# Ghostish/Open3DSOT

Measured on NVIDIA H100. Metric: template-search pairs/sec, BAT-Car fwd+bwd, higher is better.
Workload: dtype f32

## Files before the change

open3dsot_b200/csrc/pwmlp_tc.cu:

```cuda
#include "common.cuh"
#include "lift.cuh"
#include "tc_ptx.cuh"
#include "../../include/o3d_b200.h"

namespace {

struct TcAct {
    const float* x; int ld; const float* scale; const float* shift; int relu;
    struct Coef { float4 s, t; bool on; };
    template <int R> struct Batch { float4 v[R]; };
    __device__ __forceinline__ Coef prep(int k, int K) const {
        Coef c;
        c.on = k < K;
        c.s = make_float4(1.f, 1.f, 1.f, 1.f);
        c.t = make_float4(0.f, 0.f, 0.f, 0.f);
        if (c.on && scale) { c.s = ld4g(scale + k); c.t = ld4g(shift + k); }
        return c;
    }
    template <int R>
    __device__ __forceinline__ void fetch(Batch<R>& b, int p0, int stride, int P, int k, int K) const {
        const int kk = k < K ? k : 0;
#pragma unroll
        for (int i = 0; i < R; ++i) {
            const int p = p0 + i * stride;
            b.v[i] = ld4g(x + (size_t)(p < P ? p : P - 1) * ld + kk);
        }
    }
    template <int R>
    __device__ __forceinline__ float4 finish(const Batch<R>& b, const Coef& c, int i, int p, int P) const {
        float4 v = b.v[i];
        if (!(c.on && p < P)) return make_float4(0.f, 0.f, 0.f, 0.f);
        if (scale) { v.x = fmaf(v.x, c.s.x, c.t.x); v.y = fmaf(v.y, c.s.y, c.t.y); v.z = fmaf(v.z, c.s.z, c.t.z); v.w = fmaf(v.w, c.s.w, c.t.w); }
        if (relu) { v.x = fmaxf(v.x, 0.f); v.y = fmaxf(v.y, 0.f); v.z = fmaxf(v.z, 0.f); v.w = fmaxf(v.w, 0.f); }
        return v;
    }
    __device__ __forceinline__ void prefetch_rows(int p0, int rows, int P) const {
        if (p0 < P) o3d_prefetch_l2(x + (size_t)p0 * ld, (size_t)min(rows, P - p0) * ld * sizeof(float));
    }
};

struct TcLift {
    LiftView lv; const float* scale; const float* shift; int relu;
    int la;
    struct Coef { float4 s, t, u0, u1, u2, u3; bool on; };
    template <int R> struct Batch { float4 v[R]; float4 sv[R]; int nrow[R]; int tag; };
    __device__ __forceinline__ Coef prep(int k, int K) const {
        Coef c;
        c.on = k < K;
        c.s = make_float4(1.f, 1.f, 1.f, 1.f);
        c.t = c.u0 = c.u1 = c.u2 = c.u3 = make_float4(0.f, 0.f, 0.f, 0.f);
        if (c.on && scale) { c.s = ld4g(scale + k); c.t = ld4g(shift + k); }
        if (c.on && lv.u) { c.u0 = ld4g(lv.u + k); c.u1 = ld4g(lv.u + lv.ldz + k); c.u2 = ld4g(lv.u + 2 * lv.ldz + k); c.u3 = ld4g(lv.u + 3 * lv.ldz + k); }
        return c;
    }
    template <int R>
    __device__ __forceinline__ void fetch(Batch<R>& b, int p0, int stride, int P, int k, int K) const {
        const int kk = k < K ? k : 0;
        if (lv.z) {
            int row[R];
            if (b.tag == p0 + 1) {
#pragma unroll
                for (int i = 0; i < R; ++i) row[i] = b.nrow[i];
            } else if (R == 4 && stride == 1 && (p0 & 3) == 0 && p0 + 3 < P) {
                const int4 r4 = __ldg(reinterpret_cast<const int4*>(lv.gidx + p0));
                row[0] = r4.x; row[R > 1 ? 1 : 0] = r4.y; row[R > 2 ? 2 : 0] = r4.z; row[R > 3 ? 3 : 0] = r4.w;
            } else {
#pragma unroll
                for (int i = 0; i < R; ++i) {
                    const int p = p0 + i * stride;
                    row[i] = __ldg(lv.gidx + (p < P ? p : P - 1));
                }
            }
#pragma unroll
            for (int i = 0; i < R; ++i) b.v[i] = ld4g(lv.z + (size_t)row[i] * lv.ldz + kk);
            if (la == 0) {
#pragma unroll
                for (int i = 0; i < R; ++i) b.nrow[i] = row[i];
                b.tag = p0 + 1;
            } else {
                const int pn = p0 + la;
#pragma unroll
                for (int i = 0; i < R; ++i) {
                    const int p = pn + i * stride;
                    b.nrow[i] = __ldg(lv.gidx + (p < P ? p : P - 1));
                }
                b.tag = pn + 1;
            }
        }
        if (lv.s) {
#pragma unroll
            for (int i = 0; i < R; ++i) {
                const int p = p0 + i * stride;
                b.sv[i] = ld4g(lv.s + (size_t)(p < P ? p : P - 1) * 4);
            }
        }
    }
    template <int R>
    __device__ __forceinline__ float4 finish(const Batch<R>& b, const Coef& c, int i, int p, int P) const {
        const float4 zero = make_float4(0.f, 0.f, 0.f, 0.f);
        if (!(c.on && p < P)) return zero;
        float4 v = lift_val4(lv.z ? b.v[i] : zero, lv.s ? b.sv[i] : zero, c.u0, c.u1, c.u2, c.u3);
        if (scale) { v.x = fmaf(v.x, c.s.x, c.t.x); v.y = fmaf(v.y, c.s.y, c.t.y); v.z = fmaf(v.z, c.s.z, c.t.z); v.w = fmaf(v.w, c.s.w, c.t.w); }
        if (relu) { v.x = fmaxf(v.x, 0.f); v.y = fmaxf(v.y, 0.f); v.z = fmaxf(v.z, 0.f); v.w = fmaxf(v.w, 0.f); }
        return v;
    }
    __device__ __forceinline__ void prefetch_rows(int p0, int rows, int P) const {
        if (p0 >= P) return;
        const size_t n = (size_t)min(rows, P - p0);
        if (lv.z) o3d_prefetch_l2(lv.gidx + p0, n * sizeof(int32_t));
        if (lv.s) o3d_prefetch_l2(lv.s + (size_t)p0 * 4, n * 16);
    }
};

struct TcDy {
    const float* g; int ldg; const float* y; int ldy; const float* a; const float* b; const float* cc;
    const float* dpool; const int32_t* sel; int S; int ldp;
    int sh;
    int dbg;
    struct Coef { float4 a, b, c; bool on; };
    template <int R> struct Batch { float4 g[R]; float4 y[R]; bool shared; };
    __device__ __forceinline__ Coef prep(int k, int K) const {
        Coef c;
        c.on = k < K;
        c.a = make_float4(1.f, 1.f, 1.f, 1.f);
        c.b = c.c = make_float4(0.f, 0.f, 0.f, 0.f);
        if (c.on && a) { c.a = ld4g(a + k); c.b = ld4g(b + k); c.c = ld4g(cc + k); }
        return c;
    }
    template <int R>
    __device__ __forceinline__ void fetch(Batch<R>& bt, int p0, int stride, int P, int k, int K) const {
        const int kk = k < K ? k : 0;
        bt.shared = false;
        if (dpool) {
            const int pf = p0 < P ? p0 : P - 1;
            const int pe = p0 + (R - 1) * stride;
            const int pl = pe < P ? pe : P - 1;
            if (R >= 2 && (pf >> sh) == (pl >> sh)) {
                bt.shared = true;
                const size_t go = (size_t)(pf >> sh) * ldp + kk;
                if (!(dbg & 256)) {
                    bt.g[0] = ld4g(dpool + go);
                    const int4 sl = __ldg(reinterpret_cast<const int4*>(sel + go));
                    bt.g[R >= 2 ? 1 : 0] = make_float4(__int_as_float(sl.x), __int_as_float(sl.y), __int_as_float(sl.z), __int_as_float(sl.w));
                } else {
                    bt.g[0] = bt.g[R >= 2 ? 1 : 0] = make_float4(0.f, 0.f, 0.f, 0.f);
                }
            } else {
#pragma unroll
                for (int i = 0; i < R; ++i) {
                    const int p = p0 + i * stride, pp = p < P ? p : P - 1;
                    const int s = pp & (S - 1);
                    const size_t go = (size_t)(pp >> sh) * ldp + kk;
                    const int4 sl = __ldg(reinterpret_cast<const int4*>(sel + go));
                    const float4 d = ld4g(dpool + go);
                    bt.g[i] = make_float4(sl.x == s ? d.x : 0.f, sl.y == s ? d.y : 0.f, sl.z == s ? d.z : 0.f, sl.w == s ? d.w : 0.f);
                }
            }
        } else {
#pragma unroll
            for (int i = 0; i < R; ++i) {
                const int p = p0 + i * stride;
                bt.g[i] = ld4g(g + (size_t)(p < P ? p : P - 1) * ldg + kk);
            }
        }
#pragma unroll
        for (int i = 0; i < R; ++i) {
            const int p = p0 + i * stride;
            bt.y[i] = (a && !(dbg & 512)) ? ld4g(y + (size_t)(p < P ? p : P - 1) * ldy + kk) : make_float4(0.f, 0.f, 0.f, 0.f);
        }
    }
    template <int R>
    __device__ __forceinline__ float4 finish(const Batch<R>& bt, const Coef& c, int i, int p, int P) const {
        if (!(c.on && p < P)) return make_float4(0.f, 0.f, 0.f, 0.f);
        float4 v = bt.g[i];
        if (bt.shared) {
            const int s = p & (S - 1);
            const float4 d = bt.g[0], sl = bt.g[R >= 2 ? 1 : 0];
            v = make_float4(__float_as_int(sl.x) == s ? d.x : 0.f, __float_as_int(sl.y) == s ? d.y : 0.f,
                            __float_as_int(sl.z) == s ? d.z : 0.f, __float_as_int(sl.w) == s ? d.w : 0.f);
        }
        if (a) {
            const float4 yy = bt.y[i];
            v.x = fmaf(c.a.x, v.x, fmaf(c.c.x, yy.x, c.b.x)); v.y = fmaf(c.a.y, v.y, fmaf(c.c.y, yy.y, c.b.y));
            v.z = fmaf(c.a.z, v.z, fmaf(c.c.z, yy.z, c.b.z)); v.w = fmaf(c.a.w, v.w, fmaf(c.c.w, yy.w, c.b.w));
        }
        return v;
    }
    __device__ __forceinline__ void prefetch_rows(int p0, int rows, int P) const {
        if (p0 >= P) return;
        const size_t n = (size_t)min(rows, P - p0);
        if (!dpool) o3d_prefetch_l2(g + (size_t)p0 * ldg, n * ldg * sizeof(float));
        if (a) o3d_prefetch_l2(y + (size_t)p0 * ldy, n * ldy * sizeof(float));
        if (dpool) {
            const int g0 = p0 >> sh, g1 = (p0 + (int)n - 1) >> sh;
            const size_t bytes = (size_t)(g1 - g0 + 1) * ldp * sizeof(float);
            o3d_prefetch_l2(dpool + (size_t)g0 * ldp, bytes);
            o3d_prefetch_l2(sel + (size_t)g0 * ldp, bytes);
        }
    }
};

template <int LD>
struct TcFwdEpi {
    float* y; int ldy; const float* bias; double* sum; double* sumsq;
    int S, log2S; float* ymax; float* ymin; int32_t* arg; int ldp;
    float bv, mx, mn; int ax, an; double d1, d2;
    __device__ __forceinline__ void begin(int ch, int Nw) {
        d1 = d2 = 0.0;
        bv = (bias && ch < Nw) ? bias[ch] : 0.f;
        mx = -INFINITY; mn = INFINITY; ax = an = 0;
    }
    __device__ __forceinline__ void prefetch(int, int, int, int) {}
    __device__ __forceinline__ const int32_t* lift_gidx() const { return nullptr; }
    __device__ __forceinline__ const float* lift_s() const { return nullptr; }
    __device__ __forceinline__ void set_tile(const int32_t*, const float4*) {}
    __device__ __forceinline__ void group(const uint32_t (&r)[16], int ch, int Nw, int pbase, int P) {
        if (ch >= Nw) return;
        float s1 = 0.f, s2 = 0.f;
        const int smask = S - 1;
        float* yp = y ? y + (size_t)pbase * ldy + ch : nullptr;
        if (pbase + 16 <= P && (S == 0 || S >= 16)) {
            float v[16];
#pragma unroll
            for (int j = 0; j < 16; ++j) v[j] = __uint_as_float(r[j]) + bv;
            if (yp) {
                const size_t st = LD ? (size_t)LD : (size_t)ldy;
#pragma unroll
                for (int j = 0; j < 16; ++j) yp[j * st] = v[j];
            }
#pragma unroll
            for (int j = 0; j < 16; ++j) {
                s1 += v[j];
                s2 = fmaf(v[j], v[j], s2);
            }
            if (S > 0) {
                float gm = v[0], gn = v[0];
                int ga = 0, gb = 0;
#pragma unroll
                for (int j = 1; j < 16; ++j) {
                    if (v[j] > gm) { gm = v[j]; ga = j; }
                    if (v[j] < gn) { gn = v[j]; gb = j; }
                }
                const int s0 = pbase & smask;
                if (s0 == 0) { mx = gm; ax = ga; mn = gn; an = gb; }
                else {
                    if (gm > mx) { mx = gm; ax = s0 + ga; }
                    if (gn < mn) { mn = gn; an = s0 + gb; }
                }
                if (s0 + 16 == S) {
                    const size_t o = (size_t)(pbase >> log2S) * ldp + ch;
                    ymax[o] = mx; ymin[o] = mn; arg[o] = ax | (an << 16);
                }
            }
        } else {
#pragma unroll
            for (int j = 0; j < 16; ++j) {
                if (pbase + j >= P) break;
                const float v = __uint_as_float(r[j]) + bv;
                if (yp) yp[(size_t)j * ldy] = v;
                s1 += v;
                s2 = fmaf(v, v, s2);
                if (S > 0) {
                    const int s = (pbase + j) & smask;
                    if (s == 0) { mx = -INFINITY; mn = INFINITY; ax = an = 0; }
                    if (v > mx) { mx = v; ax = s; }
                    if (v < mn) { mn = v; an = s; }
                    if (s == smask) {
                        const size_t o = (size_t)((pbase + j) >> log2S) * ldp + ch;
                        ymax[o] = mx; ymin[o] = mn; arg[o] = ax | (an << 16);
                    }
                }
            }
        }
        d1 += (double)s1;
        d2 += (double)s2;
    }
    __device__ __forceinline__ void end(int ch, int Nw) {
        if (sum && ch < Nw) {
            atomicAdd(sum + ch, d1);
            atomicAdd(sumsq + ch, d2);
        }
    }
};

template <int LD, bool LIFT = false>
struct TcDgradEpi {
    float* out; int ldo; const float* yprev; int ldyp; const float* scale; const float* shift; int relu;
    double* s1g; double* s2y;
    LiftView lv;
    float sc, sh; double d1, d2;
    float yv[16];
    float u0, u1, u2, u3; const int32_t* gs; const float4* ss;
    __device__ __forceinline__ bool lifted() const { return LIFT; }
    __device__ __forceinline__ void begin(int ch, int Nw) {
        d1 = d2 = 0.0;
        sc = (scale && ch < Nw) ? scale[ch] : 1.f;
        sh = (shift && ch < Nw) ? shift[ch] : 0.f;
        if constexpr (LIFT) {
            const bool on = lv.u && ch < Nw;
            u0 = on ? lv.u[ch] : 0.f; u1 = on ? lv.u[lv.ldz + ch] : 0.f; u2 = on ? lv.u[2 * lv.ldz + ch] : 0.f; u3 = on ? lv.u[3 * lv.ldz + ch] : 0.f;
            gs = nullptr;
        }
    }
    __device__ __forceinline__ const int32_t* lift_gidx() const { return LIFT ? lv.gidx : nullptr; }
    __device__ __forceinline__ const float* lift_s() const { return LIFT ? lv.s : nullptr; }
    __device__ __forceinline__ void set_tile(const int32_t* g, const float4* s4) { if constexpr (LIFT) { gs = g; ss = s4; } }
    __device__ __forceinline__ void prefetch_lift(int ch, int pbase, int col, int P) {
#pragma unroll
        for (int j = 0; j < 16; ++j) {
            const float z = lv.z ? __ldg(lv.z + (size_t)gs[col + j] * lv.ldz + ch) : 0.f;
            const float4 sv = lv.s ? ss[col + j] : make_float4(0.f, 0.f, 0.f, 0.f);
            yv[j] = lift_val(z, sv, u0, u1, u2, u3);
        }
    }
    __device__ __forceinline__ void prefetch(int ch, int Nw, int pbase, int P) {
        if (ch >= Nw) return;
        if constexpr (LIFT) { prefetch_lift(ch, pbase, pbase & (TC_N - 1), P); return; }
        if (!yprev) return;
        if (pbase + 16 <= P) {
            const float* yp = yprev + (size_t)pbase * ldyp + ch;
            const size_t st = LD ? (size_t)LD : (size_t)ldyp;
#pragma unroll
            for (int j = 0; j < 16; ++j) yv[j] = __ldg(yp + j * st);
        } else {
#pragma unroll
            for (int j = 0; j < 16; ++j) {
                const int pj = min(pbase + j, P - 1);
                yv[j] = __ldg(yprev + (size_t)pj * ldyp + ch);
            }
        }
    }
    __device__ __forceinline__ void group(const uint32_t (&r)[16], int ch, int Nw, int pbase, int P) {
        if (ch >= Nw) return;
        float s1 = 0.f, s2 = 0.f;
        float* op = out + (size_t)pbase * ldo + ch;
        if (pbase + 16 <= P) {
            float v[16];
#pragma unroll
            for (int j = 0; j < 16; ++j) v[j] = __uint_as_float(r[j]);
            if (yprev || lifted()) {
                if (relu) {
#pragma unroll
                    for (int j = 0; j < 16; ++j) v[j] = fmaf(yv[j], sc, sh) > 0.f ? v[j] : 0.f;
                }
#pragma unroll
                for (int j = 0; j < 16; ++j) s2 = fmaf(v[j], yv[j], s2);
            }
            const size_t st = LD ? (size_t)LD : (size_t)ldo;
#pragma unroll
            for (int j = 0; j < 16; ++j) {
                s1 += v[j];
                op[j * st] = v[j];
            }
        } else {
#pragma unroll
            for (int j = 0; j < 16; ++j) {
                if (pbase + j >= P) break;
                float v = __uint_as_float(r[j]);
                if (yprev || lifted()) {
                    if (relu && !(fmaf(yv[j], sc, sh) > 0.f)) v = 0.f;
                    s2 = fmaf(v, yv[j], s2);
                }
                s1 += v;
                op[(size_t)j * ldo] = v;
            }
        }
        d1 += (double)s1;
        d2 += (double)s2;
    }
    __device__ __forceinline__ void end(int ch, int Nw) {
        if (s1g && ch < Nw) {
            atomicAdd(s1g + ch, d1);
            atomicAdd(s2y + ch, d2);
        }
    }
};

constexpr int TC_STAGES = 2;
constexpr int TC_STAGE_BYTES = 4 * TILE_BYTES;
constexpr int TC_EPI_LD = 68;
constexpr int TC_EPI_BYTES = TC_M * TC_EPI_LD * 4;
constexpr int TC_THREADS = 512;
constexpr int TC_SMEM = TC_STAGES * TC_STAGE_BYTES + 2 * TC_EPI_BYTES + 1024 + 256 + 1024 + 4096;

template <int R>
__device__ __forceinline__ void stage_acc(const float (&acc)[R], float* stg, int ld) {
    const int w = (threadIdx.x >> 5) & 3, lane = threadIdx.x & 31;
#pragma unroll
    for (int i = 0; i < R; ++i) {
        const int row = 16 * w + (lane >> 2) + 8 * ((i >> 1) & 1), col = 8 * (i >> 2) + 2 * (lane & 3) + (i & 1);
        stg[col * ld + row] = acc[i];
    }
}

template <class BLoad, class Epi>
__global__ void __launch_bounds__(TC_THREADS, 1)
    pw_tc_kernel(BLoad bl, const uint8_t* __restrict__ wtiles, int P, int K, int Nw, int nkb, Epi epi, int dbg, int rev) {
    extern __shared__ uint8_t smem_raw[];
    uint8_t* smem = reinterpret_cast<uint8_t*>((reinterpret_cast<uintptr_t>(smem_raw) + 1023) & ~(uintptr_t)1023);
    uint8_t* tail = smem + TC_STAGES * TC_STAGE_BYTES + 2 * TC_EPI_BYTES;
    uint64_t* full = reinterpret_cast<uint64_t*>(tail);
    uint64_t* empty = full + TC_STAGES;

    const int warp = threadIdx.x >> 5, lane = threadIdx.x & 31;
    const int mt0 = blockIdx.y;
    const int n_ptiles = (P + TC_N - 1) / TC_N;
    auto tile_of = [&](int t) { return rev ? n_ptiles - 1 - t : t; };

    if (threadIdx.x == 0) {
        for (int s = 0; s < TC_STAGES; ++s) {
            o3d_mbar_init(full + s, 256 + 1);
            o3d_mbar_init(empty + s, 8);
        }
        o3d_fence_mbar_init();
    }
    __syncthreads();

    if (warp < 8) {
        const int h = warp >> 2;
        const int tw = threadIdx.x & 127;
        const int ch = mt0 * TC_M + tw;
        float* stg = reinterpret_cast<float*>(smem + TC_STAGES * TC_STAGE_BYTES + h * TC_EPI_BYTES);
        int32_t* gsm = reinterpret_cast<int32_t*>(tail + 256);
        float4* ssm = reinterpret_cast<float4*>(tail + 256 + 1024);
        epi.begin(ch, Nw);
        const int Nw_e = (dbg & 4) ? 0 : Nw;
        int stage = 0, phase = 0, buf = 0;
        for (int t = blockIdx.x; t < n_ptiles; t += gridDim.x) {
            const int pt0 = tile_of(t) * TC_N;
            {
                const int32_t* gi = epi.lift_gidx();
                const float* si = epi.lift_s();
                if (gi || si) {
                    const int pp = min(pt0 + tw, P - 1);
                    if (gi && h == 0) gsm[buf * TC_N + tw] = __ldg(gi + pp);
                    if (si && h == 1) ssm[buf * TC_N + tw] = ld4g(si + (size_t)pp * 4);
                    asm volatile("bar.sync 1, 256;" ::: "memory");
                    epi.set_tile(gsm + buf * TC_N, ssm + buf * TC_N);
                }
            }
            const int pb = pt0 + h * 64;
            epi.prefetch(ch, Nw_e, pb, P);
            float acc[64];
#pragma unroll
            for (int i = 0; i < 64; ++i) acc[i] = 0.f;
            for (int kb = 0; kb < nkb; ++kb) {
                o3d_mbar_wait(full + stage, phase);
                const uint32_t sb = o3d_smem_u32(smem + stage * TC_STAGE_BYTES);
                const uint32_t xb = sb + 2 * TILE_BYTES + h * (TILE_BYTES / 2);
                wgmma_fence_acc(acc);
                wgmma_fence();
                wgmma_3xtf32_kblock<128>(acc, make_desc(xb), make_desc(xb + TILE_BYTES), make_desc(sb), make_desc(sb + TILE_BYTES),
                                         kb == 0);
                wgmma_commit();
                wgmma_wait<0>();
                wgmma_fence_acc(acc);
                if (lane == 0) o3d_mbar_arrive(empty + stage);
                if (++stage == TC_STAGES) { stage = 0; phase ^= 1; }
            }
            asm volatile("bar.sync %0, 128;" ::"r"(2 + h) : "memory");
            stage_acc(acc, stg, TC_EPI_LD);
            asm volatile("bar.sync %0, 128;" ::"r"(2 + h) : "memory");
            const float* row = stg + tw * TC_EPI_LD;
#pragma unroll 1
            for (int cg = 0; cg < 4; ++cg) {
                uint32_t r[16];
#pragma unroll
                for (int j = 0; j < 4; ++j) {
                    const float4 v = *reinterpret_cast<const float4*>(row + cg * 16 + 4 * j);
                    r[4 * j] = __float_as_uint(v.x); r[4 * j + 1] = __float_as_uint(v.y);
                    r[4 * j + 2] = __float_as_uint(v.z); r[4 * j + 3] = __float_as_uint(v.w);
                }
                epi.group(r, ch, Nw_e, pb + cg * 16, P);
                if (cg + 1 < 4) epi.prefetch(ch, Nw_e, pb + (cg + 1) * 16, P);
            }
            buf ^= 1;
        }
        epi.end(ch, Nw);
    } else {
        const int pt = (warp - 8) * 32 + lane;
        const int chunk = pt & 7;
        const int row0 = (pt >> 3) * 4;
        int stage = 0, phase = 0;
        if (dbg & 2) P = 0;
        struct Cur { int t, kb, p0; };
        auto advance = [&](Cur& c) {
            if (++c.kb == nkb) {
                c.kb = 0;
                c.t += gridDim.x;
                if (c.t < n_ptiles) c.p0 = tile_of(c.t) * TC_N;
            }
        };
        using Batch4 = typename BLoad::template Batch<4>;
        auto issue = [&](Batch4& r, typename BLoad::Coef& cf, const Cur& c) {
            if (c.t >= n_ptiles) return;
            const int k = c.kb * TC_K + chunk * 4;
            cf = bl.prep(k, K);
            if (P > 0) bl.fetch(r, c.p0 + row0, 1, P, k, K);
        };
        Cur c0{(int)blockIdx.x, 0, 0};
        if (c0.t < n_ptiles) c0.p0 = tile_of(c0.t) * TC_N;
        Batch4 r0{};
        typename BLoad::Coef f0 = bl.prep(chunk * 4, K);
        issue(r0, f0, c0);
        if (pt == 0 && c0.t < n_ptiles) bl.prefetch_rows(c0.p0, TC_N, P);
        while (c0.t < n_ptiles) {
            o3d_mbar_wait(empty + stage, phase ^ 1);
            if (pt == 0) {
                o3d_mbar_expect_tx(full + stage, 2 * TILE_BYTES);
                o3d_bulk_g2s(smem + stage * TC_STAGE_BYTES, wtiles + ((size_t)mt0 * nkb + c0.kb) * (2 * TILE_BYTES), 2 * TILE_BYTES,
                             full + stage);
                const int tn = c0.t + (int)gridDim.x;
                if (c0.kb == 0 && tn < n_ptiles) bl.prefetch_rows(tile_of(tn) * TC_N, TC_N, P);
            }
            uint8_t* xhi = smem + stage * TC_STAGE_BYTES + 2 * TILE_BYTES;
            uint8_t* xlo = xhi + TILE_BYTES;
#pragma unroll
            for (int i = 0; i < 4; ++i) {
                const float4 v = P > 0 ? bl.finish(r0, f0, i, c0.p0 + row0 + i, P) : make_float4(0.f, 0.f, 0.f, 0.f);
                const uint32_t off = sw128(row0 + i, chunk);
                *reinterpret_cast<float4*>(xhi + off) = hi_part(v);
                *reinterpret_cast<float4*>(xlo + off) = lo_part(v);
            }
            o3d_fence_proxy_async();
            o3d_mbar_arrive(full + stage);
            if (++stage == TC_STAGES) { stage = 0; phase ^= 1; }
            advance(c0);
            issue(r0, f0, c0);
        }
    }
}

constexpr int WG_STAGES = 3;
constexpr int WG_AHEAD = 4;
constexpr int WG_THREADS = 512;
constexpr int WG_SMEM = WG_STAGES * 4 * TILE_BYTES + 1024 + 256;

template <class L>
__device__ __forceinline__ void store_transposed(const L& ld, const typename L::template Batch<4>& raw, const typename L::Coef& cf,
                                                 uint8_t* hi, int c_local, int p_first, int prow0, int pend) {
#pragma unroll
    for (int i = 0; i < 4; ++i) {
        const int pl = prow0 + 8 * i;
        const float4 v = ld.finish(raw, cf, i, p_first + pl, pend);
        const float e[4] = {v.x, v.y, v.z, v.w};
#pragma unroll
        for (int j = 0; j < 4; ++j) {
            const uint32_t off = sw128(c_local + j, pl >> 2) + (uint32_t)((pl & 3) * 4);
            const float h = hi1(e[j]);
            *reinterpret_cast<float*>(hi + off) = h;
            *reinterpret_cast<float*>(hi + TILE_BYTES + off) = e[j] - h;
        }
    }
}

template <class XB>
__global__ void __launch_bounds__(WG_THREADS, 1)
    pw_wgrad_tc_kernel(TcDy da, XB xb, int P, int M, int N, int chunk, float* __restrict__ dW, int lddw, float* __restrict__ part,
                       int dbg) {
    extern __shared__ uint8_t smem_raw[];
    uint8_t* smem = reinterpret_cast<uint8_t*>((reinterpret_cast<uintptr_t>(smem_raw) + 1023) & ~(uintptr_t)1023);
    uint64_t* full = reinterpret_cast<uint64_t*>(smem + WG_STAGES * 4 * TILE_BYTES);
    uint64_t* empty = full + WG_STAGES;

    const int warp = threadIdx.x >> 5, lane = threadIdx.x & 31;
    const int m0 = blockIdx.z * TC_M, n0 = blockIdx.y * TC_N;
    const int pbeg = blockIdx.x * chunk, pend = min(P, pbeg + chunk);
    const int nkb = pend > pbeg ? (pend - pbeg + TC_K - 1) / TC_K : 0;
    auto kpos = [&](int i) { return pbeg + i * TC_K; };

    if (threadIdx.x == 0) {
        for (int s = 0; s < WG_STAGES; ++s) {
            o3d_mbar_init(full + s, 256);
            o3d_mbar_init(empty + s, 8);
        }
        o3d_fence_mbar_init();
    }
    __syncthreads();

    if (warp < 8) {
        const int h = warp >> 2, w = warp & 3;
        float acc[64];
#pragma unroll
        for (int i = 0; i < 64; ++i) acc[i] = 0.f;
        int stage = 0, phase = 0;
        for (int kb = 0; kb < nkb; ++kb) {
            o3d_mbar_wait(full + stage, phase);
            const uint32_t sb = o3d_smem_u32(smem + stage * 4 * TILE_BYTES);
            const uint32_t ab = sb + h * (TILE_BYTES / 2);
            wgmma_fence_acc(acc);
            wgmma_fence();
            if (!(dbg & 32))
                wgmma_3xtf32_kblock<128>(acc, make_desc(ab), make_desc(ab + TILE_BYTES), make_desc(sb + 2 * TILE_BYTES),
                                         make_desc(sb + 3 * TILE_BYTES), kb == 0);
            wgmma_commit();
            wgmma_wait<0>();
            wgmma_fence_acc(acc);
            if (lane == 0) o3d_mbar_arrive(empty + stage);
            if (++stage == WG_STAGES) { stage = 0; phase ^= 1; }
        }
        const int Mt = TC_M * (int)gridDim.z, Nt = TC_N * (int)gridDim.y;
        float* __restrict__ out = part ? part + (size_t)blockIdx.x * Mt * Nt : nullptr;
#pragma unroll
        for (int i = 0; i < 64; i += 4) {
#pragma unroll
            for (int rr = 0; rr < 2; ++rr) {
                const int m = m0 + h * 64 + 16 * w + (lane >> 2) + 8 * rr, n = n0 + 8 * (i >> 2) + 2 * (lane & 3);
                const float v0 = acc[i + 2 * rr], v1 = acc[i + 2 * rr + 1];
                if (out) {
                    *reinterpret_cast<float2*>(out + (size_t)m * Nt + n) = make_float2(v0, v1);
                } else if (nkb > 0 && m < M) {
                    if (n < N) atomicAdd(dW + (size_t)m * lddw + n, v0);
                    if (n + 1 < N) atomicAdd(dW + (size_t)m * lddw + n + 1, v1);
                }
            }
        }
    } else {
        const int pw = warp - 8;
        const int c4 = pw * 4 + (lane & 3), prow0 = lane >> 2;
        const bool pt0 = pw == 0 && lane == 0;
        TcDy::Batch<4> ra = {};
        typename XB::template Batch<4> rb = {};
        auto fetch = [&](int kb) {
            if (dbg & 2) return;
            da.fetch(ra, kpos(kb) + prow0, 8, pend, m0 + c4 * 4, M);
            xb.fetch(rb, kpos(kb) + prow0, 8, pend, n0 + c4 * 4, N);
        };
        auto prefetch = [&](int kb) {
            if (pt0 && kb < nkb) {
                da.prefetch_rows(kpos(kb), TC_K, pend);
                xb.prefetch_rows(kpos(kb), TC_K, pend);
            }
        };
        int stage = 0, phase = 0;
        for (int kb = 0; kb < WG_AHEAD; ++kb) prefetch(kb);
        if (nkb > 0) fetch(0);
        for (int kb = 0; kb < nkb; ++kb) {
            prefetch(kb + WG_AHEAD);
            o3d_mbar_wait(empty + stage, phase ^ 1);
            uint8_t* sbase = smem + stage * 4 * TILE_BYTES;
            store_transposed(da, ra, da.prep(m0 + c4 * 4, M), sbase, c4 * 4, kpos(kb), prow0, pend);
            store_transposed(xb, rb, xb.prep(n0 + c4 * 4, N), sbase + 2 * TILE_BYTES, c4 * 4, kpos(kb), prow0, pend);
            o3d_fence_proxy_async();
            o3d_mbar_arrive(full + stage);
            if (kb + 1 < nkb) fetch(kb + 1);
            if (++stage == WG_STAGES) { stage = 0; phase ^= 1; }
        }
    }
}

__global__ void __launch_bounds__(256)
    wgrad_reduce_kernel(const float* __restrict__ part, int splits, int Mt, int Nt, int M, int N, float* __restrict__ dW,
                        int lddw) {
    const int sub = threadIdx.x & 7;
    const int n4 = (blockIdx.x * 32 + (threadIdx.x >> 3)) * 4, m = blockIdx.y;
    float4 acc = make_float4(0.f, 0.f, 0.f, 0.f);
    if (n4 < N && m < M) {
        const float* p = part + (size_t)m * Nt + n4;
        for (int s = sub; s < splits; s += 8) {
            const float4 v = __ldg(reinterpret_cast<const float4*>(p + (size_t)s * Mt * Nt));
            acc.x += v.x; acc.y += v.y; acc.z += v.z; acc.w += v.w;
        }
    }
#pragma unroll
    for (int o = 4; o >= 1; o >>= 1) {
        acc.x += __shfl_xor_sync(0xFFFFFFFFu, acc.x, o); acc.y += __shfl_xor_sync(0xFFFFFFFFu, acc.y, o);
        acc.z += __shfl_xor_sync(0xFFFFFFFFu, acc.z, o); acc.w += __shfl_xor_sync(0xFFFFFFFFu, acc.w, o);
    }
    if (sub == 0 && n4 < N && m < M) {
        float* o = dW + (size_t)m * lddw + n4;
        o[0] += acc.x;
        if (n4 + 1 < N) o[1] += acc.y;
        if (n4 + 2 < N) o[2] += acc.z;
        if (n4 + 3 < N) o[3] += acc.w;
    }
}

__global__ void w_pretile_kernel(const float* __restrict__ W, int ld, int rows, int K, int nkb, uint8_t* __restrict__ out) {
    const int m_tile = blockIdx.y, kb = blockIdx.x;
    uint8_t* dst = out + ((size_t)m_tile * nkb + kb) * (2 * TILE_BYTES);
    for (int id = threadIdx.x; id < TC_M * 8; id += blockDim.x) {
        const int r = id >> 3, c = id & 7;
        const int row = m_tile * TC_M + r, k = kb * TC_K + c * 4;
        float4 v = make_float4(0.f, 0.f, 0.f, 0.f);
        if (row < rows && k < K) v = *reinterpret_cast<const float4*>(W + (size_t)row * ld + k);
        const uint32_t off = sw128(r, c);
        *reinterpret_cast<float4*>(dst + off) = hi_part(v);
        *reinterpret_cast<float4*>(dst + TILE_BYTES + off) = lo_part(v);
    }
}

int g_tc_debug = 0;
}
extern int o3d_g_fps_wide;
extern int o3d_g_sa_fused_dbg;
namespace {
inline int ilog2_exact(int v) { int l = 0; while ((1 << l) < v) ++l; return l; }
thread_local int g_tc_rev = 0;

template <class BLoad, class Epi>
int launch_tc(BLoad bl, const uint8_t* wtiles, int P, int K, int Nw, Epi epi, cudaStream_t st, const char* name) {
    auto kern = pw_tc_kernel<BLoad, Epi>;
    O3D_CUDA(cudaFuncSetAttribute(kern, cudaFuncAttributeMaxDynamicSharedMemorySize, TC_SMEM), name);
    const int gy = (Nw + TC_M - 1) / TC_M;
    const int nkb = (K + TC_K - 1) / TC_K;
    const int n_ptiles = (P + TC_N - 1) / TC_N;
    int gx = o3d_num_sms() / gy;
    if (gx < 1) gx = 1;
    if (gx > n_ptiles) gx = n_ptiles;
    kern<<<dim3(gx, gy), TC_THREADS, TC_SMEM, st>>>(bl, wtiles, P, K, Nw, nkb, epi, g_tc_debug, g_tc_rev);
    O3D_CHECK_LAUNCH(name);
    return O3D_OK;
}

template <int LD, class BLoad>
int launch_fwd(const BLoad& bl, const void* wtiles, const float* bias, int P, int K, int Nw, float* y, int ldy, double* sum,
               double* sumsq, int S, float* ymax, float* ymin, int32_t* arg, int ldp, cudaStream_t st) {
    TcFwdEpi<LD> ep{};
    ep.y = y; ep.ldy = ldy; ep.bias = bias; ep.sum = sum; ep.sumsq = sumsq;
    ep.S = S; ep.ymax = ymax; ep.ymin = ymin; ep.arg = arg; ep.ldp = ldp;
    ep.log2S = 0;
    while ((1 << ep.log2S) < S) ++ep.log2S;
    return launch_tc(bl, (const uint8_t*)wtiles, P, K, Nw, ep, st, "o3d_pw_fwd_tc");
}

template <int LD, bool LIFT = false>
int launch_dgrad(const TcDy& bl, const void* wtiles_t, int P, int Cout, int Cin, float* out, int ldo, const float* yprev,
                 int ldyp, const float* pscale, const float* pshift, int prelu, double* s1, double* s2y, cudaStream_t st,
                 const LiftView* lv = nullptr) {
    if constexpr (!LIFT) {
        if (lv) return launch_dgrad<LD, true>(bl, wtiles_t, P, Cout, Cin, out, ldo, yprev, ldyp, pscale, pshift, prelu, s1, s2y, st, lv);
    }
    TcDgradEpi<LD, LIFT> ep{};
    if (lv) ep.lv = *lv;
    ep.out = out; ep.ldo = ldo; ep.yprev = yprev; ep.ldyp = ldyp; ep.scale = pscale; ep.shift = pshift; ep.relu = prelu;
    ep.s1g = s1; ep.s2y = s2y;
    return launch_tc(bl, (const uint8_t*)wtiles_t, P, Cout, Cin, ep, st, "o3d_pw_dgrad_tc");
}

}

extern "C" void o3d_debug_set(int tc_debug) {
    g_tc_debug = tc_debug;
    o3d_g_no_skinny = (tc_debug & 128) != 0;
    o3d_g_fps_wide = (tc_debug & 1024) != 0;
    o3d_g_sa_fused_dbg = (tc_debug >> 11) & 15;
}
extern "C" void o3d_pw_tc_set_reverse(int rev) { g_tc_rev = rev; }

extern "C" long long o3d_pw_tc_wtile_bytes(int rows, int K) {
    const long long mt = (rows + TC_M - 1) / TC_M, nkb = (K + TC_K - 1) / TC_K;
    return mt * nkb * 2 * TILE_BYTES;
}

extern "C" int o3d_pw_tc_pretile(const float* w, int ldw, int rows, int K, void* wtiles, void* stream) {
    O3D_REQUIRE(w && wtiles, O3D_ERR_ARG, "o3d_pw_tc_pretile: null pointer");
    O3D_REQUIRE((K & 3) == 0 && (ldw & 3) == 0, O3D_ERR_ARG, "o3d_pw_tc_pretile: K and ldw must be multiples of 4");
    O3D_REQUIRE(((uintptr_t)wtiles & 15) == 0 && ((uintptr_t)w & 15) == 0, O3D_ERR_ALIGN, "o3d_pw_tc_pretile: alignment");
    const int mt = (rows + TC_M - 1) / TC_M, nkb = (K + TC_K - 1) / TC_K;
    w_pretile_kernel<<<dim3(nkb, mt), 256, 0, (cudaStream_t)stream>>>(w, ldw, rows, K, nkb, (uint8_t*)wtiles);
    O3D_CHECK_LAUNCH("o3d_pw_tc_pretile");
    return O3D_OK;
}

extern "C" int o3d_pw_fwd_tc(const float* x, int ldx, const float* in_scale, const float* in_shift, int in_relu,
                             const void* wtiles, const float* bias, int P, int K, int N, float* y, int ldy, double* sum,
                             double* sumsq, int S, float* ymax, float* ymin, int32_t* arg, int ldp, void* stream) {
    O3D_REQUIRE(x && wtiles, O3D_ERR_ARG, "o3d_pw_fwd_tc: null pointer");
    O3D_REQUIRE(P >= 0 && K >= 4 && N >= 1 && (K & 3) == 0 && (ldx & 3) == 0, O3D_ERR_ARG, "o3d_pw_fwd_tc: bad sizes");
    O3D_REQUIRE(S == 0 || (P % S == 0 && 64 % S == 0 && ymax && ymin && arg), O3D_ERR_ARG,
                "o3d_pw_fwd_tc: pooling group size must divide 64 and P");
    if (P == 0) return O3D_OK;
    const int Nw = (N + 3) & ~3;
    TcAct bl{x, ldx, in_scale, in_shift, in_relu};
    cudaStream_t st = (cudaStream_t)stream;
#define O3D_FWD_ARGS bl, wtiles, bias, P, K, Nw, y, ldy, sum, sumsq, S, ymax, ymin, arg, ldp, st
    if (ldy == 64) return launch_fwd<64>(O3D_FWD_ARGS);
    if (ldy == 128) return launch_fwd<128>(O3D_FWD_ARGS);
    if (ldy == 256) return launch_fwd<256>(O3D_FWD_ARGS);
    return launch_fwd<0>(O3D_FWD_ARGS);
#undef O3D_FWD_ARGS
}

namespace {
int dgrad_tc_impl(const float* g, int ldg, const float* y, int ldy, const float* a, const float* b, const float* cc,
                  const float* dpool, const int32_t* sel, int S, int ldp, const void* wtiles_t, int P, int Cout, int Cin,
                  float* out, int ldo, const float* yprev, int ldyp, const float* pscale, const float* pshift, int prelu,
                  double* s1, double* s2y, void* stream, const LiftView* lv) {
    O3D_REQUIRE((g || dpool) && wtiles_t && out, O3D_ERR_ARG, "o3d_pw_dgrad_tc: null pointer");
    O3D_REQUIRE((Cout & 3) == 0 && (Cin & 3) == 0, O3D_ERR_ARG, "o3d_pw_dgrad_tc: channel counts must be multiples of 4");
    if (P == 0) return O3D_OK;
    TcDy bl{g, ldg, y, ldy, a, b, cc, dpool, sel, S > 0 ? S : 1, ldp, ilog2_exact(S > 0 ? S : 1), g_tc_debug};
    cudaStream_t st = (cudaStream_t)stream;
    const int ld = (!yprev || ldyp == ldo) ? ldo : 0;
#define O3D_DG_ARGS bl, wtiles_t, P, Cout, Cin, out, ldo, yprev, ldyp, pscale, pshift, prelu, s1, s2y, st, lv
    if (ld == 64) return launch_dgrad<64>(O3D_DG_ARGS);
    if (ld == 128) return launch_dgrad<128>(O3D_DG_ARGS);
    if (ld == 256) return launch_dgrad<256>(O3D_DG_ARGS);
    return launch_dgrad<0>(O3D_DG_ARGS);
#undef O3D_DG_ARGS
}
}

extern "C" int o3d_pw_dgrad_tc(const float* g, int ldg, const float* y, int ldy, const float* a, const float* b,
                               const float* cc, const float* dpool, const int32_t* sel, int S, int ldp,
                               const void* wtiles_t, int P, int Cout, int Cin, float* out, int ldo, const float* yprev,
                               int ldyp, const float* pscale, const float* pshift, int prelu, double* s1, double* s2y,
                               void* stream) {
    return dgrad_tc_impl(g, ldg, y, ldy, a, b, cc, dpool, sel, S, ldp, wtiles_t, P, Cout, Cin, out, ldo, yprev, ldyp, pscale,
                         pshift, prelu, s1, s2y, stream, nullptr);
}

extern "C" int o3d_pw_dgrad_tc_lift(const float* g, int ldg, const float* y, int ldy, const float* a, const float* b,
                                    const float* cc, const float* dpool, const int32_t* sel, int S, int ldp,
                                    const void* wtiles_t, int P, int Cout, int Cin, float* out, int ldo,
                                    const o3d_lift_t* lf, const int32_t* gidx, const float* pscale, const float* pshift,
                                    int prelu, double* s1, double* s2y, void* stream) {
    O3D_REQUIRE(lf && (gidx || !lf->z) && (lf->z || lf->s) && lf->ldz == Cin, O3D_ERR_ARG, "o3d_pw_dgrad_tc_lift: lift descriptor");
    const LiftView lv{lf->z, lf->ldz, lf->z ? gidx : nullptr, lf->s, lf->u};
    return dgrad_tc_impl(g, ldg, y, ldy, a, b, cc, dpool, sel, S, ldp, wtiles_t, P, Cout, Cin, out, ldo, nullptr, 0, pscale,
                         pshift, prelu, s1, s2y, stream, &lv);
}

namespace {
template <class XB>
int launch_wgrad(const TcDy& da, const XB& xb, int P, int Cout, int Cin, float* dw, int lddw, float* part, long long part_floats,
                 cudaStream_t st) {
    auto kern = pw_wgrad_tc_kernel<XB>;
    const char* name = part ? "o3d_pw_wgrad_tc2" : "o3d_pw_wgrad_tc";
    O3D_CUDA(cudaFuncSetAttribute(kern, cudaFuncAttributeMaxDynamicSharedMemorySize, WG_SMEM), name);
    const int mt = (Cout + TC_M - 1) / TC_M, nt = (Cin + TC_N - 1) / TC_N;
    const int Mt = mt * TC_M, Nt = nt * TC_N;
    int splits = o3d_num_sms() / (mt * nt);
    if (splits < 1) splits = 1;
    if (part) {
        const long long cap = part_floats / ((long long)Mt * Nt);
        if (splits > cap) splits = (int)cap;
        const int by_size = (P + 127) / 128;
        if (splits > by_size) splits = by_size;
        O3D_REQUIRE(splits >= 1, O3D_ERR_ARG, "o3d_pw_wgrad_tc2: workspace too small");
    }
    int chunk = (P + splits - 1) / splits;
    chunk = ((chunk + TC_K - 1) / TC_K) * TC_K;
    splits = (P + chunk - 1) / chunk;
    kern<<<dim3(splits, nt, mt), WG_THREADS, WG_SMEM, st>>>(da, xb, P, Cout, Cin, chunk, dw, lddw, part, g_tc_debug);
    O3D_CHECK_LAUNCH(name);
    if (part) {
        dim3 rg((Cin / 4 + 31) / 32, Cout);
        wgrad_reduce_kernel<<<rg, 256, 0, st>>>(part, splits, Mt, Nt, Cout, Cin, dw, lddw);
        O3D_CHECK_LAUNCH("o3d_pw_wgrad_tc2: reduce");
    }
    return O3D_OK;
}
inline TcLift make_tclift(const o3d_lift_t* lf, const int32_t* gidx, const float* scale, const float* shift, int relu) {
    return TcLift{LiftView{lf->z, lf->ldz, lf->z ? gidx : nullptr, lf->s, lf->u}, scale, shift, relu, 0};
}
}

extern "C" int o3d_pw_wgrad_tc(const float* g, int ldg, const float* y, int ldy, const float* a, const float* b,
                               const float* cc, const float* dpool, const int32_t* sel, int S, int ldp, const float* x,
                               int ldx, const float* in_scale, const float* in_shift, int in_relu, int P, int Cout,
                               int Cin, float* dw, int lddw, void* stream) {
    O3D_REQUIRE((g || dpool) && x && dw, O3D_ERR_ARG, "o3d_pw_wgrad_tc: null pointer");
    O3D_REQUIRE((Cout & 3) == 0 && (Cin & 3) == 0 && (ldx & 3) == 0, O3D_ERR_ARG,
                "o3d_pw_wgrad_tc: channel counts / leading dimensions must be multiples of 4");
    if (P == 0) return O3D_OK;
    TcDy da{g, ldg, y, ldy, a, b, cc, dpool, sel, S > 0 ? S : 1, ldp, ilog2_exact(S > 0 ? S : 1), g_tc_debug};
    TcAct xb{x, ldx, in_scale, in_shift, in_relu};
    return launch_wgrad(da, xb, P, Cout, Cin, dw, lddw, nullptr, 0, (cudaStream_t)stream);
}

extern "C" long long o3d_pw_wgrad_tc2_workspace_floats(void) {
    return (long long)o3d_num_sms() * TC_M * TC_N;
}

extern "C" int o3d_pw_wgrad_tc2(const float* g, int ldg, const float* y, int ldy, const float* a, const float* b,
                                const float* cc, const float* dpool, const int32_t* sel, int S, int ldp, const float* x,
                                int ldx, const float* in_scale, const float* in_shift, int in_relu, int P, int Cout,
                                int Cin, float* dw, int lddw, float* part, long long part_floats, void* stream) {
    O3D_REQUIRE((g || dpool) && x && dw && part, O3D_ERR_ARG, "o3d_pw_wgrad_tc2: null pointer");
    O3D_REQUIRE((Cout & 3) == 0 && (Cin & 3) == 0 && (ldx & 3) == 0 && (lddw & 3) == 0, O3D_ERR_ARG,
                "o3d_pw_wgrad_tc2: channel counts / leading dimensions must be multiples of 4");
    if (P == 0) return O3D_OK;
    TcDy da{g, ldg, y, ldy, a, b, cc, dpool, sel, S > 0 ? S : 1, ldp, ilog2_exact(S > 0 ? S : 1), g_tc_debug};
    TcAct xb{x, ldx, in_scale, in_shift, in_relu};
    return launch_wgrad(da, xb, P, Cout, Cin, dw, lddw, part, part_floats, (cudaStream_t)stream);
}

extern "C" int o3d_pw_wgrad_tc_lift(const float* g, int ldg, const float* y, int ldy, const float* a, const float* b,
                                    const float* cc, const float* dpool, const int32_t* sel, int S, int ldp,
                                    const o3d_lift_t* lf, const int32_t* gidx, const float* in_scale, const float* in_shift,
                                    int in_relu, int P, int Cout, int Cin, float* dw, int lddw, float* part,
                                    long long part_floats, void* stream) {
    O3D_REQUIRE((g || dpool) && lf && (gidx || !lf->z) && dw, O3D_ERR_ARG, "o3d_pw_wgrad_tc_lift: null pointer");
    O3D_REQUIRE((Cout & 3) == 0 && (Cin & 3) == 0 && lf->ldz == Cin && (lddw & 3) == 0, O3D_ERR_ARG,
                "o3d_pw_wgrad_tc_lift: channel counts / leading dimensions");
    if (P == 0) return O3D_OK;
    TcDy da{g, ldg, y, ldy, a, b, cc, dpool, sel, S > 0 ? S : 1, ldp, ilog2_exact(S > 0 ? S : 1), g_tc_debug};
    TcLift xb = make_tclift(lf, gidx, in_scale, in_shift, in_relu);
    xb.la = TC_K;
    return launch_wgrad(da, xb, P, Cout, Cin, dw, lddw, part, part_floats, (cudaStream_t)stream);
}

extern "C" int o3d_pw_fwd_tc_lift(const o3d_lift_t* lf, const int32_t* gidx, const float* in_scale, const float* in_shift,
                                  int in_relu, const void* wtiles, const float* bias, int P, int K, int N, float* y, int ldy,
                                  double* sum, double* sumsq, int S, float* ymax, float* ymin, int32_t* arg, int ldp,
                                  void* stream) {
    O3D_REQUIRE(lf && (gidx || !lf->z) && wtiles, O3D_ERR_ARG, "o3d_pw_fwd_tc_lift: null pointer");
    O3D_REQUIRE(P >= 0 && K >= 32 && N >= 1 && (K & 3) == 0 && lf->ldz == K, O3D_ERR_ARG, "o3d_pw_fwd_tc_lift: bad sizes");
    O3D_REQUIRE(S == 0 || (P % S == 0 && 64 % S == 0 && ymax && ymin && arg), O3D_ERR_ARG,
                "o3d_pw_fwd_tc_lift: pooling group size must divide 64 and P");
    if (P == 0) return O3D_OK;
    const int Nw = (N + 3) & ~3;
    const TcLift bl = make_tclift(lf, gidx, in_scale, in_shift, in_relu);
    cudaStream_t st = (cudaStream_t)stream;
#define O3D_FWD_ARGS bl, wtiles, bias, P, K, Nw, y, ldy, sum, sumsq, S, ymax, ymin, arg, ldp, st
    if (ldy == 64) return launch_fwd<64>(O3D_FWD_ARGS);
    if (ldy == 128) return launch_fwd<128>(O3D_FWD_ARGS);
    if (ldy == 256) return launch_fwd<256>(O3D_FWD_ARGS);
    return launch_fwd<0>(O3D_FWD_ARGS);
#undef O3D_FWD_ARGS
}
```

open3dsot_b200/csrc/tc_ptx.cuh:

```cuda
#pragma once
#include "common.cuh"

namespace {

constexpr int TC_M = 128;
constexpr int TC_N = 128;
constexpr int TC_K = 32;
constexpr int TILE_BYTES = TC_M * TC_K * 4;

__device__ __forceinline__ void wgmma_fence() { asm volatile("wgmma.fence.sync.aligned;" ::: "memory"); }
__device__ __forceinline__ void wgmma_commit() { asm volatile("wgmma.commit_group.sync.aligned;" ::: "memory"); }
template <int N>
__device__ __forceinline__ void wgmma_wait() { asm volatile("wgmma.wait_group.sync.aligned %0;" ::"n"(N) : "memory"); }
template <int R>
__device__ __forceinline__ void wgmma_fence_acc(float (&d)[R]) {
#pragma unroll
    for (int i = 0; i < R; ++i) asm volatile("" : "+f"(d[i])::"memory");
}

__device__ __forceinline__ void wgmma_tf32_n64(float (&d)[32], uint64_t adesc, uint64_t bdesc, uint32_t accumulate) {
    asm volatile(
        "{\n\t.reg .pred p;\n\t"
        "setp.ne.b32 p, %34, 0;\n\t"
        "wgmma.mma_async.sync.aligned.m64n64k8.f32.tf32.tf32 "
        "{%0, %1, %2, %3, %4, %5, %6, %7, %8, %9, %10, %11, %12, %13, %14, %15, %16, %17, %18, %19, %20, %21, %22, %23, %24, %25, %26, %27, %28, %29, %30, %31}, "
        "%32, %33, p, 1, 1;\n\t}"
        : "+f"(d[0]), "+f"(d[1]), "+f"(d[2]), "+f"(d[3]), "+f"(d[4]), "+f"(d[5]), "+f"(d[6]), "+f"(d[7]), "+f"(d[8]), "+f"(d[9]), "+f"(d[10]), "+f"(d[11]), "+f"(d[12]), "+f"(d[13]), "+f"(d[14]), "+f"(d[15]), "+f"(d[16]), "+f"(d[17]), "+f"(d[18]), "+f"(d[19]), "+f"(d[20]), "+f"(d[21]), "+f"(d[22]), "+f"(d[23]), "+f"(d[24]), "+f"(d[25]), "+f"(d[26]), "+f"(d[27]), "+f"(d[28]), "+f"(d[29]), "+f"(d[30]), "+f"(d[31])
        : "l"(adesc), "l"(bdesc), "r"(accumulate)
        : "memory");
}

__device__ __forceinline__ void wgmma_tf32_n128(float (&d)[64], uint64_t adesc, uint64_t bdesc, uint32_t accumulate) {
    asm volatile(
        "{\n\t.reg .pred p;\n\t"
        "setp.ne.b32 p, %66, 0;\n\t"
        "wgmma.mma_async.sync.aligned.m64n128k8.f32.tf32.tf32 "
        "{%0, %1, %2, %3, %4, %5, %6, %7, %8, %9, %10, %11, %12, %13, %14, %15, %16, %17, %18, %19, %20, %21, %22, %23, %24, %25, %26, %27, %28, %29, %30, %31, %32, %33, %34, %35, %36, %37, %38, %39, %40, %41, %42, %43, %44, %45, %46, %47, %48, %49, %50, %51, %52, %53, %54, %55, %56, %57, %58, %59, %60, %61, %62, %63}, "
        "%64, %65, p, 1, 1;\n\t}"
        : "+f"(d[0]), "+f"(d[1]), "+f"(d[2]), "+f"(d[3]), "+f"(d[4]), "+f"(d[5]), "+f"(d[6]), "+f"(d[7]), "+f"(d[8]), "+f"(d[9]), "+f"(d[10]), "+f"(d[11]), "+f"(d[12]), "+f"(d[13]), "+f"(d[14]), "+f"(d[15]), "+f"(d[16]), "+f"(d[17]), "+f"(d[18]), "+f"(d[19]), "+f"(d[20]), "+f"(d[21]), "+f"(d[22]), "+f"(d[23]), "+f"(d[24]), "+f"(d[25]), "+f"(d[26]), "+f"(d[27]), "+f"(d[28]), "+f"(d[29]), "+f"(d[30]), "+f"(d[31]), "+f"(d[32]), "+f"(d[33]), "+f"(d[34]), "+f"(d[35]), "+f"(d[36]), "+f"(d[37]), "+f"(d[38]), "+f"(d[39]), "+f"(d[40]), "+f"(d[41]), "+f"(d[42]), "+f"(d[43]), "+f"(d[44]), "+f"(d[45]), "+f"(d[46]), "+f"(d[47]), "+f"(d[48]), "+f"(d[49]), "+f"(d[50]), "+f"(d[51]), "+f"(d[52]), "+f"(d[53]), "+f"(d[54]), "+f"(d[55]), "+f"(d[56]), "+f"(d[57]), "+f"(d[58]), "+f"(d[59]), "+f"(d[60]), "+f"(d[61]), "+f"(d[62]), "+f"(d[63])
        : "l"(adesc), "l"(bdesc), "r"(accumulate)
        : "memory");
}


__device__ __forceinline__ uint64_t make_desc(uint32_t smem_addr) {
    uint64_t d = 0;
    d |= (uint64_t)((smem_addr >> 4) & 0x3FFF);
    d |= (uint64_t)1 << 16;
    d |= (uint64_t)(1024 >> 4) << 32;
    d |= (uint64_t)1 << 62;
    return d;
}

__device__ __host__ __forceinline__ uint32_t sw128(int r, int c) {
    return (uint32_t)((r >> 3) * 1024 + (r & 7) * 128 + ((c ^ (r & 7)) << 4));
}

__device__ __forceinline__ float hi1(float x) { return __uint_as_float(__float_as_uint(x) & 0xFFFFE000u); }
__device__ __forceinline__ float4 hi_part(const float4& v) { return make_float4(hi1(v.x), hi1(v.y), hi1(v.z), hi1(v.w)); }
__device__ __forceinline__ float4 lo_part(const float4& v) {
    return make_float4(v.x - hi1(v.x), v.y - hi1(v.y), v.z - hi1(v.z), v.w - hi1(v.w));
}
__device__ __forceinline__ float4 ld4g(const float* p) { return __ldg(reinterpret_cast<const float4*>(p)); }

template <int N>
__device__ __forceinline__ void wgmma_3xtf32_kblock(float (&d)[N / 2], uint64_t ahi, uint64_t alo, uint64_t bhi, uint64_t blo,
                                                    bool first) {
#pragma unroll
    for (int ks = 0; ks < TC_K / 8; ++ks) {
        const uint64_t adv = (uint64_t)((ks * 32) >> 4);
        if constexpr (N == 64) {
            wgmma_tf32_n64(d, alo + adv, bhi + adv, (first && ks == 0) ? 0u : 1u);
            wgmma_tf32_n64(d, ahi + adv, blo + adv, 1u);
            wgmma_tf32_n64(d, ahi + adv, bhi + adv, 1u);
        } else {
            wgmma_tf32_n128(d, alo + adv, bhi + adv, (first && ks == 0) ? 0u : 1u);
            wgmma_tf32_n128(d, ahi + adv, blo + adv, 1u);
            wgmma_tf32_n128(d, ahi + adv, bhi + adv, 1u);
        }
    }
}

}
```

Baseline: 2762.

## Split activations in registers, defer epilogue into next tile's wgmma loop

The producer now stores raw fp32 activation tiles into padded shared memory instead of pre-split hi/lo swizzled tiles. Consumers load A fragments into registers, split them into hi/lo there, and issue register-sourced wgmma with one group kept in flight. The epilogue for the previous tile is deferred and interleaved with the next tile's MMA loop, the pipeline grows to three stages, and setmaxnreg rebalances registers between consumer and producer warps. This aims to halve the A-tile shared memory traffic and producer work and to hide epilogue cost behind tensor-core work, at the price of higher register pressure and more complex ordering of the barriers.

```diff
diff --git a/open3dsot_b200/csrc/pwmlp_tc.cu b/open3dsot_b200/csrc/pwmlp_tc.cu
--- a/open3dsot_b200/csrc/pwmlp_tc.cu
+++ b/open3dsot_b200/csrc/pwmlp_tc.cu
@@ -202,6 +202,7 @@
 
 template <int LD>
 struct TcFwdEpi {
+    static constexpr bool kDefer = true;
     float* y; int ldy; const float* bias; double* sum; double* sumsq;
     int S, log2S; float* ymax; float* ymin; int32_t* arg; int ldp;
     float bv, mx, mn; int ax, an; double d1, d2;
@@ -285,6 +286,7 @@
 
 template <int LD, bool LIFT = false>
 struct TcDgradEpi {
+    static constexpr bool kDefer = !LIFT;
     float* out; int ldo; const float* yprev; int ldyp; const float* scale; const float* shift; int relu;
     double* s1g; double* s2y;
     LiftView lv;
@@ -376,12 +378,19 @@
     }
 };
 
-constexpr int TC_STAGES = 2;
-constexpr int TC_STAGE_BYTES = 4 * TILE_BYTES;
+constexpr int TC_STAGES = 3;
+constexpr int TC_XLD = TC_K + 4;
+constexpr int TC_XBYTES = TC_N * TC_XLD * 4;
+constexpr int TC_STAGE_BYTES = 2 * TILE_BYTES + TC_XBYTES;
+static_assert(TC_STAGE_BYTES % 1024 == 0, "stage size");
 constexpr int TC_EPI_LD = 68;
 constexpr int TC_EPI_BYTES = TC_M * TC_EPI_LD * 4;
 constexpr int TC_THREADS = 512;
-constexpr int TC_SMEM = TC_STAGES * TC_STAGE_BYTES + 2 * TC_EPI_BYTES + 1024 + 256 + 1024 + 4096;
+constexpr int TC_SLICES = 3;
+constexpr int TC_SMEM = TC_STAGES * TC_STAGE_BYTES + 2 * TC_EPI_BYTES + 1024 + 256 + TC_SLICES * TC_N * (4 + 16);
+static_assert(TC_SMEM <= 227 * 1024, "pw_tc_kernel shared memory");
+constexpr int TC_CONSUMER_REGS = 152, TC_PRODUCER_REGS = 104;
+static_assert(TC_THREADS / 2 * (TC_CONSUMER_REGS + TC_PRODUCER_REGS) <= 65536, "register file");
 
 template <int R>
 __device__ __forceinline__ void stage_acc(const float (&acc)[R], float* stg, int ld) {
@@ -417,15 +426,30 @@
     __syncthreads();
 
     if (warp < 8) {
+        asm volatile("setmaxnreg.inc.sync.aligned.u32 %0;" ::"n"(TC_CONSUMER_REGS));
         const int h = warp >> 2;
         const int tw = threadIdx.x & 127;
         const int ch = mt0 * TC_M + tw;
         float* stg = reinterpret_cast<float*>(smem + TC_STAGES * TC_STAGE_BYTES + h * TC_EPI_BYTES);
         int32_t* gsm = reinterpret_cast<int32_t*>(tail + 256);
-        float4* ssm = reinterpret_cast<float4*>(tail + 256 + 1024);
+        float4* ssm = reinterpret_cast<float4*>(tail + 256 + TC_SLICES * TC_N * 4);
         epi.begin(ch, Nw);
         const int Nw_e = (dbg & 4) ? 0 : Nw;
         int stage = 0, phase = 0, buf = 0;
+        int pend = 0, ppb = 0;
+        const float* row = stg + tw * TC_EPI_LD;
+        auto epi_group = [&]() {
+            const int cg = 4 - pend;
+            uint32_t r[16];
+#pragma unroll
+            for (int j = 0; j < 4; ++j) {
+                const float4 v = *reinterpret_cast<const float4*>(row + cg * 16 + 4 * j);
+                r[4 * j] = __float_as_uint(v.x); r[4 * j + 1] = __float_as_uint(v.y);
+                r[4 * j + 2] = __float_as_uint(v.z); r[4 * j + 3] = __float_as_uint(v.w);
+            }
+            epi.group(r, ch, Nw_e, ppb + cg * 16, P);
+            if (--pend > 0) epi.prefetch(ch, Nw_e, ppb + (cg + 1) * 16, P);
+        };
         for (int t = blockIdx.x; t < n_ptiles; t += gridDim.x) {
             const int pt0 = tile_of(t) * TC_N;
             {
@@ -436,48 +460,76 @@
                     if (gi && h == 0) gsm[buf * TC_N + tw] = __ldg(gi + pp);
                     if (si && h == 1) ssm[buf * TC_N + tw] = ld4g(si + (size_t)pp * 4);
                     asm volatile("bar.sync 1, 256;" ::: "memory");
-                    epi.set_tile(gsm + buf * TC_N, ssm + buf * TC_N);
                 }
             }
             const int pb = pt0 + h * 64;
-            epi.prefetch(ch, Nw_e, pb, P);
+            if constexpr (!Epi::kDefer) {
+                epi.set_tile(gsm + buf * TC_N, ssm + buf * TC_N);
+                epi.prefetch(ch, Nw_e, pb, P);
+            }
             float acc[64];
 #pragma unroll
             for (int i = 0; i < 64; ++i) acc[i] = 0.f;
+            uint32_t ahi[2][4], alo[2][4];
+            const int frag = (h * 64 + 16 * (warp & 3) + (lane >> 2)) * TC_XLD + (lane & 3);
+            int prev = -1;
             for (int kb = 0; kb < nkb; ++kb) {
                 o3d_mbar_wait(full + stage, phase);
                 const uint32_t sb = o3d_smem_u32(smem + stage * TC_STAGE_BYTES);
-                const uint32_t xb = sb + 2 * TILE_BYTES + h * (TILE_BYTES / 2);
-                wgmma_fence_acc(acc);
-                wgmma_fence();
-                wgmma_3xtf32_kblock<128>(acc, make_desc(xb), make_desc(xb + TILE_BYTES), make_desc(sb), make_desc(sb + TILE_BYTES),
-                                         kb == 0);
-                wgmma_commit();
-                wgmma_wait<0>();
-                wgmma_fence_acc(acc);
-                if (lane == 0) o3d_mbar_arrive(empty + stage);
+                const float* xs = reinterpret_cast<const float*>(smem + stage * TC_STAGE_BYTES + 2 * TILE_BYTES) + frag;
+                const uint64_t bhi = make_desc(sb), blo = make_desc(sb + TILE_BYTES);
+#pragma unroll
+                for (int ks = 0; ks < TC_K / 8; ++ks) {
+                    const int b = ks & 1;
+                    const float x[4] = {xs[8 * ks], xs[8 * TC_XLD + 8 * ks], xs[8 * ks + 4], xs[8 * TC_XLD + 8 * ks + 4]};
+#pragma unroll
+                    for (int i = 0; i < 4; ++i) {
+                        const float hv = hi1(x[i]);
+                        ahi[b][i] = __float_as_uint(hv);
+                        alo[b][i] = __float_as_uint(x[i] - hv);
+                    }
+                    const uint64_t adv = (uint64_t)((ks * 32) >> 4);
+                    wgmma_fence_frag(ahi[b]);
+                    wgmma_fence_frag(alo[b]);
+                    wgmma_fence_acc(acc);
+                    wgmma_fence();
+                    wgmma_tf32_n128_rs(acc, alo[b], bhi + adv, (kb == 0 && ks == 0) ? 0u : 1u);
+                    wgmma_tf32_n128_rs(acc, ahi[b], blo + adv, 1u);
+                    wgmma_tf32_n128_rs(acc, ahi[b], bhi + adv, 1u);
+                    wgmma_commit();
+                    if (ks == 1 && pend > 0) epi_group();
+                    wgmma_wait<1>();
+                    wgmma_fence_frag(ahi[b ^ 1]);
+                    wgmma_fence_frag(alo[b ^ 1]);
+                    if (ks == 0 && prev >= 0) {
+                        if (lane == 0) o3d_mbar_arrive(empty + prev);
+                        prev = -1;
+                    }
+                }
+                prev = stage;
                 if (++stage == TC_STAGES) { stage = 0; phase ^= 1; }
             }
+            while (pend > 0) epi_group();
+            wgmma_wait<0>();
+            wgmma_fence_acc(acc);
+            if (prev >= 0 && lane == 0) o3d_mbar_arrive(empty + prev);
             asm volatile("bar.sync %0, 128;" ::"r"(2 + h) : "memory");
             stage_acc(acc, stg, TC_EPI_LD);
             asm volatile("bar.sync %0, 128;" ::"r"(2 + h) : "memory");
-            const float* row = stg + tw * TC_EPI_LD;
-#pragma unroll 1
-            for (int cg = 0; cg < 4; ++cg) {
-                uint32_t r[16];
-#pragma unroll
-                for (int j = 0; j < 4; ++j) {
-                    const float4 v = *reinterpret_cast<const float4*>(row + cg * 16 + 4 * j);
-                    r[4 * j] = __float_as_uint(v.x); r[4 * j + 1] = __float_as_uint(v.y);
-                    r[4 * j + 2] = __float_as_uint(v.z); r[4 * j + 3] = __float_as_uint(v.w);
-                }
-                epi.group(r, ch, Nw_e, pb + cg * 16, P);
-                if (cg + 1 < 4) epi.prefetch(ch, Nw_e, pb + (cg + 1) * 16, P);
-            }
-            buf ^= 1;
-        }
+            ppb = pb;
+            pend = 4;
+            if constexpr (Epi::kDefer) {
+                epi.set_tile(gsm + buf * TC_N, ssm + buf * TC_N);
+                epi.prefetch(ch, Nw_e, ppb, P);
+            } else {
+                while (pend > 0) epi_group();
+            }
+            if (++buf == TC_SLICES) buf = 0;
+        }
+        while (pend > 0) epi_group();
         epi.end(ch, Nw);
     } else {
+        asm volatile("setmaxnreg.dec.sync.aligned.u32 %0;" ::"n"(TC_PRODUCER_REGS));
         const int pt = (warp - 8) * 32 + lane;
         const int chunk = pt & 7;
         const int row0 = (pt >> 3) * 4;
@@ -513,16 +565,12 @@
                 const int tn = c0.t + (int)gridDim.x;
                 if (c0.kb == 0 && tn < n_ptiles) bl.prefetch_rows(tile_of(tn) * TC_N, TC_N, P);
             }
-            uint8_t* xhi = smem + stage * TC_STAGE_BYTES + 2 * TILE_BYTES;
-            uint8_t* xlo = xhi + TILE_BYTES;
+            float* xt = reinterpret_cast<float*>(smem + stage * TC_STAGE_BYTES + 2 * TILE_BYTES) + row0 * TC_XLD + chunk * 4;
 #pragma unroll
             for (int i = 0; i < 4; ++i) {
                 const float4 v = P > 0 ? bl.finish(r0, f0, i, c0.p0 + row0 + i, P) : make_float4(0.f, 0.f, 0.f, 0.f);
-                const uint32_t off = sw128(row0 + i, chunk);
-                *reinterpret_cast<float4*>(xhi + off) = hi_part(v);
-                *reinterpret_cast<float4*>(xlo + off) = lo_part(v);
-            }
-            o3d_fence_proxy_async();
+                *reinterpret_cast<float4*>(xt + i * TC_XLD) = v;
+            }
             o3d_mbar_arrive(full + stage);
             if (++stage == TC_STAGES) { stage = 0; phase ^= 1; }
             advance(c0);
diff --git a/open3dsot_b200/csrc/tc_ptx.cuh b/open3dsot_b200/csrc/tc_ptx.cuh
--- a/open3dsot_b200/csrc/tc_ptx.cuh
+++ b/open3dsot_b200/csrc/tc_ptx.cuh
@@ -42,6 +42,22 @@
         : "memory");
 }
 
+__device__ __forceinline__ void wgmma_tf32_n128_rs(float (&d)[64], const uint32_t (&a)[4], uint64_t bdesc, uint32_t accumulate) {
+    asm volatile(
+        "{\n\t.reg .pred p;\n\t"
+        "setp.ne.b32 p, %69, 0;\n\t"
+        "wgmma.mma_async.sync.aligned.m64n128k8.f32.tf32.tf32 "
+        "{%0, %1, %2, %3, %4, %5, %6, %7, %8, %9, %10, %11, %12, %13, %14, %15, %16, %17, %18, %19, %20, %21, %22, %23, %24, %25, %26, %27, %28, %29, %30, %31, %32, %33, %34, %35, %36, %37, %38, %39, %40, %41, %42, %43, %44, %45, %46, %47, %48, %49, %50, %51, %52, %53, %54, %55, %56, %57, %58, %59, %60, %61, %62, %63}, "
+        "{%64, %65, %66, %67}, %68, p, 1, 1;\n\t}"
+        : "+f"(d[0]), "+f"(d[1]), "+f"(d[2]), "+f"(d[3]), "+f"(d[4]), "+f"(d[5]), "+f"(d[6]), "+f"(d[7]), "+f"(d[8]), "+f"(d[9]), "+f"(d[10]), "+f"(d[11]), "+f"(d[12]), "+f"(d[13]), "+f"(d[14]), "+f"(d[15]), "+f"(d[16]), "+f"(d[17]), "+f"(d[18]), "+f"(d[19]), "+f"(d[20]), "+f"(d[21]), "+f"(d[22]), "+f"(d[23]), "+f"(d[24]), "+f"(d[25]), "+f"(d[26]), "+f"(d[27]), "+f"(d[28]), "+f"(d[29]), "+f"(d[30]), "+f"(d[31]), "+f"(d[32]), "+f"(d[33]), "+f"(d[34]), "+f"(d[35]), "+f"(d[36]), "+f"(d[37]), "+f"(d[38]), "+f"(d[39]), "+f"(d[40]), "+f"(d[41]), "+f"(d[42]), "+f"(d[43]), "+f"(d[44]), "+f"(d[45]), "+f"(d[46]), "+f"(d[47]), "+f"(d[48]), "+f"(d[49]), "+f"(d[50]), "+f"(d[51]), "+f"(d[52]), "+f"(d[53]), "+f"(d[54]), "+f"(d[55]), "+f"(d[56]), "+f"(d[57]), "+f"(d[58]), "+f"(d[59]), "+f"(d[60]), "+f"(d[61]), "+f"(d[62]), "+f"(d[63])
+        : "r"(a[0]), "r"(a[1]), "r"(a[2]), "r"(a[3]), "l"(bdesc), "r"(accumulate)
+        : "memory");
+}
+template <int R>
+__device__ __forceinline__ void wgmma_fence_frag(uint32_t (&a)[R]) {
+#pragma unroll
+    for (int i = 0; i < R; ++i) asm volatile("" : "+r"(a[i])::"memory");
+}
 
 __device__ __forceinline__ uint64_t make_desc(uint32_t smem_addr) {
     uint64_t d = 0;
```

After: 2882, median of 6. +4.3%, better.
